# friendlymatthew/heif

Hardware: AMD Instinct MI355X
Metric: Mpixels/s decoded (bit-exact) on 4032x3024 HEIC batch (higher is better)
Workload: dtype u8

## Files before the change

### heif_amd/csrc/kernels/loopfilter.hip

```cpp
#include "kernels.hpp"

#include <algorithm>
#include <string>

namespace hg {

namespace {

__constant__ uint8_t c_beta[52] = {0,  0,  0,  0,  0,  0,  0,  0,  0,  0,  0,  0,  0,  0,  0,  0,  6,  7,
                                   8,  9,  10, 11, 12, 13, 14, 15, 16, 17, 18, 20, 22, 24, 26, 28, 30, 32,
                                   34, 36, 38, 40, 42, 44, 46, 48, 50, 52, 54, 56, 58, 60, 62, 64};
__constant__ uint8_t c_tc[54] = {0, 0, 0, 0, 0, 0, 0, 0, 0, 0, 0, 0, 0, 0, 0, 0, 0, 0, 1, 1, 1, 1, 1, 1, 1, 1, 1,
                                 2, 2, 2, 2, 3, 3, 3, 3, 4, 4, 4, 5, 5, 6, 6, 7, 8, 9, 10, 11, 13, 14, 16, 18, 20, 22, 24};

__device__ __forceinline__ int clip3(int lo, int hi, int v) { return v < lo ? lo : (v > hi ? hi : v); }

struct FastDiv {
    int d;
    float r;
    __device__ __forceinline__ explicit FastDiv(int d_) : d(d_ > 0 ? d_ : 1), r(1.0f / (float)(d_ > 0 ? d_ : 1)) {}
    __device__ __forceinline__ int div(int t, int &rem) const {
        int q = (int)((float)t * r);
        rem = t - q * d;
        if (rem < 0) {
            --q;
            rem += d;
        } else if (rem >= d) {
            ++q;
            rem -= d;
        }
        return q;
    }
};

__device__ __forceinline__ int chroma_qp_map(int qpi, int chroma) {
    if (chroma != 1) return qpi < 51 ? qpi : 51;
    if (qpi < 30) return qpi;
    if (qpi > 43) return qpi - 6;
    constexpr int t[14] = {29, 30, 31, 32, 33, 33, 34, 34, 35, 35, 36, 36, 37, 37};
    return t[qpi - 30];
}

template <typename Pel>
__device__ void luma_segment(Pel *q, int sx, int sk, int qpP, int qpQ, bool nofp, bool nofq, int beta_off,
                             int tc_off, int bd) {
#define PS(i, k) q[(k) * sk - ((i) + 1) * sx]
#define QS(i, k) q[(k) * sk + (i) * sx]
    const int qpl = (qpQ + qpP + 1) >> 1;
    const int beta = c_beta[clip3(0, 51, qpl + (beta_off << 1))] * (1 << (bd - 8));
    const int tc = c_tc[clip3(0, 53, qpl + 2 + (tc_off << 1))] * (1 << (bd - 8));
    const int dp0 = abs(PS(2, 0) - 2 * PS(1, 0) + PS(0, 0)), dp3 = abs(PS(2, 3) - 2 * PS(1, 3) + PS(0, 3));
    const int dq0 = abs(QS(2, 0) - 2 * QS(1, 0) + QS(0, 0)), dq3 = abs(QS(2, 3) - 2 * QS(1, 3) + QS(0, 3));
    const int dpq0 = dp0 + dq0, dpq3 = dp3 + dq3, dp = dp0 + dp3, dq = dq0 + dq3;
    if (dpq0 + dpq3 >= beta) return;
    auto dsam = [&](int k, int dpq) {
        return dpq < (beta >> 2) && abs(PS(3, k) - PS(0, k)) + abs(QS(0, k) - QS(3, k)) < (beta >> 3) &&
               abs(PS(0, k) - QS(0, k)) < ((5 * tc + 1) >> 1);
    };
    const bool strong = dsam(0, 2 * dpq0) && dsam(3, 2 * dpq3);
    const bool dEp = dp < ((beta + (beta >> 1)) >> 3), dEq = dq < ((beta + (beta >> 1)) >> 3);
    const int maxv = (1 << bd) - 1;
    for (int k = 0; k < 4; ++k) {
        const int p0 = PS(0, k), p1 = PS(1, k), p2 = PS(2, k), p3 = PS(3, k);
        const int q0 = QS(0, k), q1 = QS(1, k), q2 = QS(2, k), q3 = QS(3, k);
        if (strong) {
            if (!nofp) {
                PS(0, k) = (Pel)clip3(p0 - 2 * tc, p0 + 2 * tc, (p2 + 2 * p1 + 2 * p0 + 2 * q0 + q1 + 4) >> 3);
                PS(1, k) = (Pel)clip3(p1 - 2 * tc, p1 + 2 * tc, (p2 + p1 + p0 + q0 + 2) >> 2);
                PS(2, k) = (Pel)clip3(p2 - 2 * tc, p2 + 2 * tc, (2 * p3 + 3 * p2 + p1 + p0 + q0 + 4) >> 3);
            }
            if (!nofq) {
                QS(0, k) = (Pel)clip3(q0 - 2 * tc, q0 + 2 * tc, (p1 + 2 * p0 + 2 * q0 + 2 * q1 + q2 + 4) >> 3);
                QS(1, k) = (Pel)clip3(q1 - 2 * tc, q1 + 2 * tc, (p0 + q0 + q1 + q2 + 2) >> 2);
                QS(2, k) = (Pel)clip3(q2 - 2 * tc, q2 + 2 * tc, (p0 + q0 + q1 + 3 * q2 + 2 * q3 + 4) >> 3);
            }
        } else {
            int delta = (9 * (q0 - p0) - 3 * (q1 - p1) + 8) >> 4;
            if (abs(delta) < tc * 10) {
                delta = clip3(-tc, tc, delta);
                if (!nofp) PS(0, k) = (Pel)clip3(0, maxv, p0 + delta);
                if (!nofq) QS(0, k) = (Pel)clip3(0, maxv, q0 - delta);
                if (dEp && !nofp)
                    PS(1, k) = (Pel)clip3(0, maxv, p1 + clip3(-(tc >> 1), tc >> 1, (((p2 + p0 + 1) >> 1) - p1 + delta) >> 1));
                if (dEq && !nofq)
                    QS(1, k) = (Pel)clip3(0, maxv, q1 + clip3(-(tc >> 1), tc >> 1, (((q2 + q0 + 1) >> 1) - q1 - delta) >> 1));
            }
        }
    }
#undef PS
#undef QS
}

}

template <typename Pel>
__global__ void __launch_bounds__(256) k_assemble(BatchArgs a) {
    const int pic = a.pic0 + blockIdx.y;
    const PicDesc pd = a.pics[pic];
    if (!(pd.flags & PD_ASSEMBLY)) return;
    const SeqParams sp = a.seqs[pd.seq];
    const int W = sp.width, H = sp.height, w4 = (W + 3) >> 2, h4 = (H + 3) >> 2;
    const int wctb = (W + (1 << sp.log2_ctb) - 1) >> sp.log2_ctb;
    const int sx = chroma_sx(sp.chroma_format), sy = chroma_sy(sp.chroma_format);
    const int cw = sp.chroma_format ? W >> sx : 0, ch = sp.chroma_format ? H >> sy : 0;
    Pel *dY = reinterpret_cast<Pel *>(a.recon + pd.recon_off);
    uint8_t *dmap = a.maps + pd.map_off;
    const int tid = blockIdx.x * blockDim.x + threadIdx.x, nth = gridDim.x * blockDim.x;
    for (uint32_t c = 0; c < pd.nchild; ++c) {
        const PicDesc cd = a.pics[pd.child0 + c];
        const SeqParams cs = a.seqs[cd.seq];
        const int cW = cs.width, cH = cs.height, cw4 = (cW + 3) >> 2, ch4 = (cH + 3) >> 2;
        const int ccw = cs.chroma_format ? cW >> sx : 0, cch = cs.chroma_format ? cH >> sy : 0;
        const Pel *sY = reinterpret_cast<const Pel *>(a.recon + cd.recon_off);
        const int nl = cW * cH, nc = ccw * cch;
        for (int t = tid; t < nl + 2 * nc; t += nth) {
            if (t < nl) {
                const int x = t % cW, y = t / cW;
                dY[(size_t)(cd.org_y + y) * W + cd.org_x + x] = sY[t];
            } else {
                const int u = t - nl, k = u / nc, v = u % nc, x = v % ccw, y = v / ccw;
                dY[(size_t)W * H + (size_t)k * cw * ch + (size_t)((cd.org_y >> sy) + y) * cw + (cd.org_x >> sx) + x] = sY[t];
            }
        }
        const uint8_t *smap = a.maps + cd.map_off;
        const int nm = cw4 * ch4;
        for (int t = tid; t < 2 * nm; t += nth) {
            const int k = t / nm, v = t % nm, x = v % cw4, y = v / cw4;
            dmap[(size_t)k * w4 * h4 + (size_t)((cd.org_y >> 2) + y) * w4 + (cd.org_x >> 2) + x] = smap[t];
        }
        const int cwctb = (cW + (1 << cs.log2_ctb) - 1) >> cs.log2_ctb;
        const int chctb = (cH + (1 << cs.log2_ctb) - 1) >> cs.log2_ctb;
        const bool sao = cd.sao_luma || cd.sao_chroma;
        for (int t = tid; t < cwctb * chctb * 8; t += nth) {
            const int b = t >> 3, x = b % cwctb, y = b / cwctb;
            uint32_t *dst = reinterpret_cast<uint32_t *>(
                a.sao + pd.sao_off + (size_t)((cd.org_y >> sp.log2_ctb) + y) * wctb + (cd.org_x >> sp.log2_ctb) + x);
            dst[t & 7] = sao ? reinterpret_cast<const uint32_t *>(a.sao + cd.sao_off + b)[t & 7] : 0u;
        }
    }
    (void)h4;
}

template <typename Pel, bool VERT>
__global__ void __launch_bounds__(256) k_deblock(BatchArgs a) {
    const int pic = a.pic0 + blockIdx.y;
    const PicDesc pd = a.pics[pic];
    if (pd.dbk_disabled || (pd.flags & PD_CHILD)) return;
    const SeqParams sp = a.seqs[pd.seq];
    const int W = sp.width, H = sp.height;
    const int w4 = (W + 3) >> 2, h4 = (H + 3) >> 2;
    const int8_t *qpy = reinterpret_cast<const int8_t *>(a.maps + pd.map_off);
    const uint8_t *flg = a.maps + pd.map_off + (size_t)w4 * h4;
    Pel *Y = reinterpret_cast<Pel *>(a.recon + pd.recon_off);
    const int sx = chroma_sx(sp.chroma_format), sy = chroma_sy(sp.chroma_format);
    const int cw = sp.chroma_format ? W >> sx : 0, ch = sp.chroma_format ? H >> sy : 0;
    const int ne_l = VERT ? (W - 1) >> 3 : (H - 1) >> 3;
    const int ns_l = VERT ? H >> 2 : W >> 2;
    const int nl = ne_l * ns_l;
    const int ne_c = VERT ? (cw - 1) >> 3 : (ch - 1) >> 3;
    const int lc = VERT ? 4 >> sy : 4 >> sx;
    const int ns_c = VERT ? ch / lc : cw / lc;
    const int nc = sp.chroma_format ? ne_c * ns_c : 0;
    const int total = nl + 2 * nc;
    const FastDiv dl(VERT ? ne_l : ns_l), dc(nc), dce(VERT ? ne_c : ns_c);
    for (int t = blockIdx.x * blockDim.x + threadIdx.x; t < total; t += gridDim.x * blockDim.x) {
        if (t < nl) {
            int x, y, tr;
            const int tq = dl.div(t, tr);
            if (VERT) {
                x = 8 * (tr + 1);
                y = 4 * tq;
            } else {
                x = 4 * tr;
                y = 8 * (tq + 1);
            }
            const int fq = flg[(y >> 2) * w4 + (x >> 2)];
            if (!(fq & (VERT ? MF_EDGE_V : MF_EDGE_H))) continue;
            const int xp = VERT ? x - 1 : x, yp = VERT ? y : y - 1;
            const int fp = flg[(yp >> 2) * w4 + (xp >> 2)];
            luma_segment<Pel>(Y + (size_t)y * W + x, VERT ? 1 : W, VERT ? W : 1, qpy[(yp >> 2) * w4 + (xp >> 2)],
                              qpy[(y >> 2) * w4 + (x >> 2)], fp & MF_NOFILT, fq & MF_NOFILT, pd.beta_off, pd.tc_off,
                              sp.bit_depth_y);
        } else {
            const int u = t - nl;
            int v, vr;
            const int cidx = 1 + dc.div(u, v);
            const int vq = dce.div(v, vr);
            int xc, yc;
            if (VERT) {
                xc = 8 * (vr + 1);
                yc = lc * vq;
            } else {
                xc = lc * vr;
                yc = 8 * (vq + 1);
            }
            const int xl = xc << sx, yl = yc << sy;
            const int fq = flg[(yl >> 2) * w4 + (xl >> 2)];
            if (!(fq & (VERT ? MF_EDGE_V : MF_EDGE_H))) continue;
            const int xlp = VERT ? xl - 1 : xl, ylp = VERT ? yl : yl - 1;
            const int fp = flg[(ylp >> 2) * w4 + (xlp >> 2)];
            const int qpP = qpy[(ylp >> 2) * w4 + (xlp >> 2)], qpQ = qpy[(yl >> 2) * w4 + (xl >> 2)];
            const int off = cidx == 1 ? sp.cb_qp_offset : sp.cr_qp_offset;
            const int qpc = chroma_qp_map(((qpQ + qpP + 1) >> 1) + off, sp.chroma_format);
            const int bd = sp.bit_depth_c;
            const int tc = c_tc[clip3(0, 53, qpc + 2 + (pd.tc_off << 1))] * (1 << (bd - 8));
            const int maxv = (1 << bd) - 1;
            Pel *C = Y + (size_t)W * H + (size_t)(cidx - 1) * cw * ch;
            Pel *q = C + (size_t)yc * cw + xc;
            const int sa = VERT ? 1 : cw, sk = VERT ? cw : 1;
            for (int k = 0; k < lc; ++k) {
                const int p0 = q[k * sk - sa], p1 = q[k * sk - 2 * sa], q0 = q[k * sk], q1 = q[k * sk + sa];
                const int delta = clip3(-tc, tc, ((((q0 - p0) * 4) + p1 - q1 + 4) >> 3));
                if (!(fp & MF_NOFILT)) q[k * sk - sa] = (Pel)clip3(0, maxv, p0 + delta);
                if (!(fq & MF_NOFILT)) q[k * sk] = (Pel)clip3(0, maxv, q0 - delta);
            }
        }
    }
}

template <typename Pel>
__device__ __forceinline__ int sao_sample(const Pel *P, int PW, int PH, int xs, int ys, int cidx, int subx,
                                          int suby, const SaoParams *sao, int wctb, int log2ctb, const uint8_t *flg,
                                          int w4, int bd) {
    int v = P[(size_t)ys * PW + xs];
    const SaoParams &s = sao[(ys >> (log2ctb - suby)) * wctb + (xs >> (log2ctb - subx))];
    const int type = s.type[cidx];
    if (!type || (flg[((ys << suby) >> 2) * w4 + ((xs << subx) >> 2)] & MF_NOFILT)) return v;
    int o = 0;
    if (type == 2) {
        const int cl = s.band_eo[cidx];
        const int hx = cl == 0 ? 1 : (cl == 1 ? 0 : (cl == 2 ? 1 : -1));
        const int vy = cl == 0 ? 0 : 1;
        const int ax = xs - hx, ay = ys - vy, bx = xs + hx, by = ys + vy;
        if (ax >= 0 && ay >= 0 && ax < PW && ay < PH && bx >= 0 && by >= 0 && bx < PW && by < PH) {
            const int na = P[(size_t)ay * PW + ax], nb = P[(size_t)by * PW + bx];
            int e = 2 + (v > na) - (v < na) + (v > nb) - (v < nb);
            if (e <= 2) e = e == 2 ? 0 : e + 1;
            o = e ? s.off[cidx][e - 1] : 0;
        }
    } else {
        const int band = v >> (bd - 5);
        const int k = (band - s.band_eo[cidx]) & 31;
        o = k < 4 ? s.off[cidx][k] : 0;
    }
    return clip3(0, (1 << bd) - 1, v + o);
}

template <typename Pel>
struct QuadLoad;
template <>
struct QuadLoad<uint8_t> {
    using W = uint32_t;
    static __device__ __forceinline__ int at(W w, int j) { return (int)((w >> (8 * j)) & 0xffu); }
};
template <>
struct QuadLoad<uint16_t> {
    using W = uint64_t;
    static __device__ __forceinline__ int at(W w, int j) { return (int)((w >> (16 * j)) & 0xffffu); }
};

template <typename Pel>
__device__ __forceinline__ bool sao_quad(const Pel *P, int PW, int PH, int xs0, int ys, int cidx, int subx, int suby,
                                         const SaoParams *sao, int wctb, int log2ctb, const uint8_t *flg, int w4,
                                         int bd, int v[4]) {
    using Q = QuadLoad<Pel>;
    using W = typename Q::W;
    const Pel *row = P + (size_t)ys * PW;
    if ((xs0 & 3) || (PW & 3) || (reinterpret_cast<uintptr_t>(row + xs0) & (sizeof(W) - 1))) return false;
    const W c = *reinterpret_cast<const W *>(row + xs0);
#pragma unroll
    for (int j = 0; j < 4; ++j) v[j] = Q::at(c, j);
    const SaoParams &s = sao[(ys >> (log2ctb - suby)) * wctb + (xs0 >> (log2ctb - subx))];
    const int type = s.type[cidx];
    if (!type) return true;
    const uint8_t *fr = flg + (size_t)((ys << suby) >> 2) * w4;
    const int b0 = (xs0 << subx) >> 2, b3 = ((xs0 + 3) << subx) >> 2;
    const int f0 = fr[b0], f3 = fr[b3];
    const int cl = s.band_eo[cidx];
    const int maxv = (1 << bd) - 1;
    int o[4] = {0, 0, 0, 0};
    if (type == 2) {
        const int hx = cl == 0 ? 1 : (cl == 1 ? 0 : (cl == 2 ? 1 : -1)), vy = cl == 0 ? 0 : 1;
        const int ya = ys - vy, yb = ys + vy;
        const bool va = ya >= 0, vb = yb < PH;
        const Pel *ra = P + (size_t)(va ? ya : ys) * PW, *rb = P + (size_t)(vb ? yb : ys) * PW;
        const W qa = *reinterpret_cast<const W *>(ra + xs0), qb = *reinterpret_cast<const W *>(rb + xs0);
        const int xa_out = hx > 0 ? xs0 - 1 : xs0 + 4, xb_out = hx > 0 ? xs0 + 4 : xs0 - 1;
        const int ea = hx != 0 && xa_out >= 0 && xa_out < PW ? (int)ra[xa_out] : 0;
        const int eb = hx != 0 && xb_out >= 0 && xb_out < PW ? (int)rb[xb_out] : 0;
#pragma unroll
        for (int j = 0; j < 4; ++j) {
            const int ja = j - hx, jb = j + hx;
            const int na = ja < 0 || ja > 3 ? ea : Q::at(qa, ja < 0 ? 0 : (ja > 3 ? 3 : ja));
            const int nb = jb < 0 || jb > 3 ? eb : Q::at(qb, jb < 0 ? 0 : (jb > 3 ? 3 : jb));
            const bool in = va && vb && xs0 + ja >= 0 && xs0 + ja < PW && xs0 + jb >= 0 && xs0 + jb < PW;
            int e = 2 + (v[j] > na) - (v[j] < na) + (v[j] > nb) - (v[j] < nb);
            e = e <= 2 ? (e == 2 ? 0 : e + 1) : e;
            o[j] = in && e ? s.off[cidx][e - 1] : 0;
        }
    } else {
#pragma unroll
        for (int j = 0; j < 4; ++j) {
            const int k = ((v[j] >> (bd - 5)) - cl) & 31;
            o[j] = k < 4 ? s.off[cidx][k] : 0;
        }
    }
#pragma unroll
    for (int j = 0; j < 4; ++j) {
        const bool nf = ((((xs0 + j) << subx) >> 2) == b0 ? f0 : f3) & MF_NOFILT;
        if (!nf) v[j] = clip3(0, maxv, v[j] + o[j]);
    }
    return true;
}

template <typename Pel>
__global__ void __launch_bounds__(256) k_sao_out(BatchArgs a) {
    const int pic = a.pic0 + blockIdx.y;
    const PicDesc pd = a.pics[pic];
    if (pd.flags & PD_CHILD) return;
    const SeqParams sp = a.seqs[pd.seq];
    const OutImage oi = a.outs[pd.image];
    const int W = sp.width, H = sp.height, log2ctb = sp.log2_ctb;
    const int wctb = (W + (1 << log2ctb) - 1) >> log2ctb;
    const int w4 = (W + 3) >> 2, h4 = (H + 3) >> 2;
    const uint8_t *flg = a.maps + pd.map_off + (size_t)w4 * h4;
    const Pel *Y = reinterpret_cast<const Pel *>(a.recon + pd.recon_off);
    const int sx = chroma_sx(sp.chroma_format), sy = chroma_sy(sp.chroma_format);
    const int cw = sp.chroma_format ? W >> sx : 0, ch = sp.chroma_format ? H >> sy : 0;
    const SaoParams *sao = a.sao + pd.sao_off;
    const int vw = min(sp.out_w, oi.width - pd.out_x), vh = min(sp.out_h, oi.height - pd.out_y);
    if (vw <= 0 || vh <= 0) return;
    const int vcw = sp.chroma_format ? (vw + (1 << sx) - 1) >> sx : 0;
    const int vch = sp.chroma_format ? (vh + (1 << sy) - 1) >> sy : 0;
    const int qw = (vw + 3) >> 2, qcw = (vcw + 3) >> 2;
    const int nl = qw * vh, nc = qcw * vch;
    const int total = nl + 2 * nc;
    const FastDiv dq(qw), dn(nc), dqc(qcw);
    for (int t = blockIdx.x * blockDim.x + threadIdx.x; t < total; t += gridDim.x * blockDim.x) {
        int cidx, q, y;
        if (t < nl) {
            cidx = 0;
            y = dq.div(t, q);
        } else {
            const int u = t - nl;
            int v;
            cidx = 1 + dn.div(u, v);
            y = dqc.div(v, q);
        }
        const int subx = cidx ? sx : 0, suby = cidx ? sy : 0;
        const int PW = cidx ? cw : W, PH = cidx ? ch : H;
        const int vwc = cidx ? vcw : vw;
        const Pel *P = cidx == 0 ? Y : Y + (size_t)W * H + (size_t)(cidx - 1) * cw * ch;
        const int x0 = q * 4, n = min(4, vwc - x0);
        const int ys = y + (sp.conf_t >> suby), xs0 = x0 + (sp.conf_l >> subx);
        const bool on = pd.sao_luma || pd.sao_chroma;
        const int bd = cidx ? sp.bit_depth_c : sp.bit_depth_y;
        int v[4];
        if (!(n == 4 && on && sao_quad(P, PW, PH, xs0, ys, cidx, subx, suby, sao, wctb, log2ctb, flg, w4, bd, v))) {
#pragma unroll
            for (int j = 0; j < 4; ++j) {
                v[j] = 0;
                if (j < n)
                    v[j] = on ? sao_sample(P, PW, PH, xs0 + j, ys, cidx, subx, suby, sao, wctb, log2ctb, flg, w4, bd)
                              : (int)P[(size_t)ys * PW + xs0 + j];
            }
        }
        const uint64_t plane = cidx == 0 ? oi.plane[0] : (cidx == 1 ? oi.plane[1] : oi.plane[2]);
        const int pitch = cidx == 0 ? oi.pitch[0] : (cidx == 1 ? oi.pitch[1] : oi.pitch[2]);
        const int ox = (pd.out_x >> subx) + x0, oy = (pd.out_y >> suby) + y;
        Pel *dst = reinterpret_cast<Pel *>(plane + (size_t)oy * pitch) + ox;
        if (n == 4 && (reinterpret_cast<uintptr_t>(dst) & (4 * sizeof(Pel) - 1)) == 0) {
            if (sizeof(Pel) == 1)
                *reinterpret_cast<uint32_t *>(dst) = (uint32_t)v[0] | (uint32_t)v[1] << 8 | (uint32_t)v[2] << 16 |
                                                     (uint32_t)v[3] << 24;
            else
                *reinterpret_cast<uint64_t *>(dst) = (uint64_t)v[0] | (uint64_t)v[1] << 16 | (uint64_t)v[2] << 32 |
                                                     (uint64_t)v[3] << 48;
        } else {
            for (int j = 0; j < n; ++j) dst[j] = (Pel)v[j];
        }
    }
}


#if defined(HG_HOST_EMU)
void emu_deblock(const BatchArgs &a) {
    if (a.has_assembly) {
        if (a.bytes_per_sample == 1) emu_launch(k_assemble<uint8_t>, 1, a.n_pics, 1, a, true);
        else emu_launch(k_assemble<uint16_t>, 1, a.n_pics, 1, a, true);
    }
    if (a.bytes_per_sample == 1) {
        emu_launch(k_deblock<uint8_t, true>, 1, a.n_pics, 1, a, true);
        emu_launch(k_deblock<uint8_t, false>, 1, a.n_pics, 1, a, true);
    } else {
        emu_launch(k_deblock<uint16_t, true>, 1, a.n_pics, 1, a, true);
        emu_launch(k_deblock<uint16_t, false>, 1, a.n_pics, 1, a, true);
    }
}
void emu_sao_out(const BatchArgs &a) {
    if (a.bytes_per_sample == 1) emu_launch(k_sao_out<uint8_t>, 1, a.n_pics, 1, a, true);
    else emu_launch(k_sao_out<uint16_t>, 1, a.n_pics, 1, a, true);
}
#else
static int lf_blocks(int forced, int n_pics, int total, int lo, int hi) {
    int v = forced > 0 ? forced : total / (n_pics > 0 ? n_pics : 1);
    if (forced <= 0) v = v < lo ? lo : (v > hi ? hi : v);
    return v < 1 ? 1 : (v > 1024 ? 1024 : v);
}
static int env_int(const char *var) {
    const char *e = std::getenv(var);
    return e ? std::atoi(e) : 0;
}

hipError_t launch_deblock(const BatchArgs &a, hipStream_t s) {
    static const int forced = env_int("HEIFGPU_DBK_BLOCKS");
    dim3 grid(lf_blocks(forced, a.n_pics, 8192, 2, 64), a.n_pics), block(256);
    if (a.has_assembly) {
        if (a.bytes_per_sample == 1) hipLaunchKernelGGL(k_assemble<uint8_t>, grid, block, 0, s, a);
        else hipLaunchKernelGGL(k_assemble<uint16_t>, grid, block, 0, s, a);
    }
    if (a.bytes_per_sample == 1) {
        hipLaunchKernelGGL((k_deblock<uint8_t, true>), grid, block, 0, s, a);
        hipLaunchKernelGGL((k_deblock<uint8_t, false>), grid, block, 0, s, a);
    } else {
        hipLaunchKernelGGL((k_deblock<uint16_t, true>), grid, block, 0, s, a);
        hipLaunchKernelGGL((k_deblock<uint16_t, false>), grid, block, 0, s, a);
    }
    return hipGetLastError();
}

hipError_t launch_sao_out(const BatchArgs &a, hipStream_t s) {
    static const int forced = env_int("HEIFGPU_SAO_BLOCKS");
    dim3 grid(lf_blocks(forced, a.n_pics, 24576, 4, 256), a.n_pics), block(256);
    if (a.bytes_per_sample == 1) hipLaunchKernelGGL(k_sao_out<uint8_t>, grid, block, 0, s, a);
    else hipLaunchKernelGGL(k_sao_out<uint16_t>, grid, block, 0, s, a);
    return hipGetLastError();
}

__global__ void __launch_bounds__(256) k_status_fold(const uint32_t *__restrict__ st, uint32_t *__restrict__ sticky,
                                                     int n) {
    const int i = blockIdx.x * 256 + threadIdx.x;
    if (i < n) {
        const uint32_t v = st[i];
        if (v) sticky[i] |= v;
    }
}

hipError_t launch_status_fold(const uint32_t *status, uint32_t *sticky, int n, hipStream_t s) {
    if (n <= 0) return hipSuccess;
    hipLaunchKernelGGL(k_status_fold, dim3((n + 255) / 256), dim3(256), 0, s, status, sticky, n);
    return hipGetLastError();
}
#endif

}
```

Before: 28190.

## Vectorize SAO output kernel with 16-byte groups and packed 16-bit SIMD math

Rewrites the SAO-and-output kernel so each thread handles a 16-byte group of samples instead of 4 samples. It uses 128-bit loads and stores and packed 2x16-bit arithmetic through v_perm table lookups. The loop now runs per plane with a strided walk that avoids per-item division, and falls back to the old quad path for unaligned or tail columns. It also adds launch_bounds occupancy 8. The bit-exact edge and band offset logic now lives in new packed code, which adds correctness risk at picture edges and for the no-filter flags.

```diff
diff --git a/heif_amd/csrc/kernels/lf_pack.hpp b/heif_amd/csrc/kernels/lf_pack.hpp
--- /dev/null
+++ b/heif_amd/csrc/kernels/lf_pack.hpp
@@ -0,0 +1,115 @@
+#pragma once
+#include "wave.hpp"
+
+namespace hg {
+namespace lfp {
+
+#if !defined(HG_HOST_EMU)
+typedef short lf_s2 __attribute__((ext_vector_type(2)));
+typedef unsigned short lf_u2 __attribute__((ext_vector_type(2)));
+template <class V>
+__device__ __forceinline__ V lf_as(uint32_t a) {
+    V v;
+    __builtin_memcpy(&v, &a, 4);
+    return v;
+}
+template <class V>
+__device__ __forceinline__ uint32_t lf_word(V v) {
+    uint32_t a;
+    __builtin_memcpy(&a, &v, 4);
+    return a;
+}
+#endif
+
+__device__ __forceinline__ uint32_t pk_add(uint32_t a, uint32_t b) {
+#if defined(HG_HOST_EMU)
+    return ((a + b) & 0xffffu) | ((((a >> 16) + (b >> 16)) & 0xffffu) << 16);
+#else
+    return lf_word(lf_as<lf_u2>(a) + lf_as<lf_u2>(b));
+#endif
+}
+__device__ __forceinline__ uint32_t pk_sub(uint32_t a, uint32_t b) {
+#if defined(HG_HOST_EMU)
+    return ((a - b) & 0xffffu) | ((((a >> 16) - (b >> 16)) & 0xffffu) << 16);
+#else
+    return lf_word(lf_as<lf_u2>(a) - lf_as<lf_u2>(b));
+#endif
+}
+__device__ __forceinline__ uint32_t pk_max_i16(uint32_t a, uint32_t b) {
+#if defined(HG_HOST_EMU)
+    const int al = (int16_t)(a & 0xffffu), ah = (int16_t)(a >> 16), bl = (int16_t)(b & 0xffffu), bh = (int16_t)(b >> 16);
+    return (uint32_t)((al > bl ? al : bl) & 0xffff) | ((uint32_t)((ah > bh ? ah : bh) & 0xffff) << 16);
+#else
+    return lf_word(__builtin_elementwise_max(lf_as<lf_s2>(a), lf_as<lf_s2>(b)));
+#endif
+}
+__device__ __forceinline__ uint32_t pk_min_i16(uint32_t a, uint32_t b) {
+#if defined(HG_HOST_EMU)
+    const int al = (int16_t)(a & 0xffffu), ah = (int16_t)(a >> 16), bl = (int16_t)(b & 0xffffu), bh = (int16_t)(b >> 16);
+    return (uint32_t)((al < bl ? al : bl) & 0xffff) | ((uint32_t)((ah < bh ? ah : bh) & 0xffff) << 16);
+#else
+    return lf_word(__builtin_elementwise_min(lf_as<lf_s2>(a), lf_as<lf_s2>(b)));
+#endif
+}
+__device__ __forceinline__ uint32_t pk_ashr(uint32_t a, int n) {
+#if defined(HG_HOST_EMU)
+    const int al = (int16_t)(a & 0xffffu), ah = (int16_t)(a >> 16);
+    return (uint32_t)((al >> n) & 0xffff) | ((uint32_t)((ah >> n) & 0xffff) << 16);
+#else
+    return lf_word(lf_as<lf_s2>(a) >> (lf_s2){(short)n, (short)n});
+#endif
+}
+__device__ __forceinline__ uint32_t pk_lshr(uint32_t a, int n) {
+#if defined(HG_HOST_EMU)
+    return ((a & 0xffffu) >> n) | (((a >> 16) >> n) << 16);
+#else
+    return lf_word(lf_as<lf_u2>(a) >> (lf_u2){(unsigned short)n, (unsigned short)n});
+#endif
+}
+
+__device__ __forceinline__ uint32_t perm(uint32_t s0, uint32_t s1, uint32_t sel) {
+#if defined(HG_HOST_EMU)
+    const uint64_t in = ((uint64_t)s0 << 32) | s1;
+    uint32_t r = 0;
+    for (int k = 0; k < 4; ++k) {
+        const uint32_t s = (sel >> (8 * k)) & 0xffu;
+        uint32_t b;
+        if (s >= 13) b = 0xffu;
+        else if (s == 12) b = 0;
+        else if (s >= 8) b = ((in >> (16 * (s - 8) + 15)) & 1) ? 0xffu : 0u;
+        else b = (uint32_t)(in >> (8 * s)) & 0xffu;
+        r |= b << (8 * k);
+    }
+    return r;
+#else
+    return __builtin_amdgcn_perm(s0, s1, sel);
+#endif
+}
+
+__device__ __forceinline__ uint32_t pk_sign_diff(uint32_t a, uint32_t b) {
+    return pk_max_i16(pk_min_i16(pk_sub(a, b), 0x00010001u), 0xffffffffu);
+}
+
+__device__ __forceinline__ uint32_t pk_from_bytes(uint32_t w, int half) {
+    return perm(0, w, half ? 0x0c030c02u : 0x0c010c00u);
+}
+__device__ __forceinline__ uint32_t pk_to_bytes(uint32_t p0, uint32_t p1) { return perm(p1, p0, 0x06040200u); }
+
+__device__ __forceinline__ void sao_tables(uint32_t d1, uint32_t d2, uint32_t d3, bool edge, uint32_t &lo, uint32_t &hi) {
+    if (edge) {
+        lo = perm(d1, d2, 0x020c0006u);
+        hi = d3 & 0xffu;
+    } else {
+        lo = perm(d1, d2, 0x0c020006u) | (d3 << 24);
+        hi = 0;
+    }
+}
+__device__ __forceinline__ uint32_t sao_lookup(uint32_t lo, uint32_t hi, uint32_t idx) {
+    return pk_ashr(perm(hi, lo, (idx << 8) | 0x000c000cu), 8);
+}
+__device__ __forceinline__ uint32_t pk_add_clip(uint32_t c, uint32_t o, uint32_t maxv2) {
+    return pk_min_i16(pk_max_i16(pk_add(c, o), 0), maxv2);
+}
+
+}
+}
diff --git a/heif_amd/csrc/kernels/loopfilter.hip b/heif_amd/csrc/kernels/loopfilter.hip
--- a/heif_amd/csrc/kernels/loopfilter.hip
+++ b/heif_amd/csrc/kernels/loopfilter.hip
@@ -1,4 +1,5 @@
 #include "kernels.hpp"
+#include "lf_pack.hpp"
 
 #include <algorithm>
 #include <string>
@@ -314,7 +315,132 @@
 }
 
 template <typename Pel>
-__global__ void __launch_bounds__(256) k_sao_out(BatchArgs a) {
+__device__ __forceinline__ void sao_out_quad(const Pel *P, int PW, int PH, int xs0, int ys, int n, bool on, int cidx,
+                                             int subx, int suby, const SaoParams *sao, int wctb, int log2ctb,
+                                             const uint8_t *flg, int w4, int bd, Pel *dst) {
+    int v[4];
+    if (!(n == 4 && on && sao_quad(P, PW, PH, xs0, ys, cidx, subx, suby, sao, wctb, log2ctb, flg, w4, bd, v))) {
+#pragma unroll
+        for (int j = 0; j < 4; ++j) {
+            v[j] = 0;
+            if (j < n)
+                v[j] = on ? sao_sample(P, PW, PH, xs0 + j, ys, cidx, subx, suby, sao, wctb, log2ctb, flg, w4, bd)
+                          : (int)P[(size_t)ys * PW + xs0 + j];
+        }
+    }
+    if (n == 4 && (reinterpret_cast<uintptr_t>(dst) & (4 * sizeof(Pel) - 1)) == 0) {
+        if (sizeof(Pel) == 1)
+            *reinterpret_cast<uint32_t *>(dst) = (uint32_t)v[0] | (uint32_t)v[1] << 8 | (uint32_t)v[2] << 16 |
+                                                 (uint32_t)v[3] << 24;
+        else
+            *reinterpret_cast<uint64_t *>(dst) = (uint64_t)v[0] | (uint64_t)v[1] << 16 | (uint64_t)v[2] << 32 |
+                                                 (uint64_t)v[3] << 48;
+    } else {
+        for (int j = 0; j < n; ++j) dst[j] = (Pel)v[j];
+    }
+}
+
+struct alignas(16) Vec16 {
+    uint32_t w[4];
+};
+__device__ __forceinline__ Vec16 load16(const void *p) {
+    Vec16 v;
+    __builtin_memcpy(&v, __builtin_assume_aligned(p, 16), 16);
+    return v;
+}
+__device__ __forceinline__ void store16(void *p, const Vec16 &v) {
+    __builtin_memcpy(__builtin_assume_aligned(p, 16), &v, 16);
+}
+
+template <typename Pel>
+__device__ __forceinline__ uint32_t pack_of(const Vec16 &v, int p) {
+    if constexpr (sizeof(Pel) == 1) return lfp::pk_from_bytes(v.w[p >> 1], p & 1);
+    else return v.w[p];
+}
+
+template <typename Pel>
+__device__ __forceinline__ void sao_group(const Pel *P, int PW, int PH, int xs0, int ys, int cidx, int subx, int suby,
+                                          const SaoParams *sao, int wctb, int log2ctb, const uint8_t *flg, int w4,
+                                          int bd, Vec16 &out) {
+    using namespace lfp;
+    constexpr int G = 16 / (int)sizeof(Pel), BITS = 8 * (int)sizeof(Pel);
+    constexpr int NP = G / 2;
+    const Pel *row = P + (size_t)ys * PW + xs0;
+    const Vec16 c = load16(row);
+    out = c;
+    const uint32_t *sw =
+        reinterpret_cast<const uint32_t *>(sao + (ys >> (log2ctb - suby)) * wctb + (xs0 >> (log2ctb - subx)));
+    const uint64_t head = (uint64_t)sw[0] | (uint64_t)sw[1] << 32;
+    const int type = (int)(int8_t)(head >> (8 * cidx));
+    if (!type) return;
+    const int cl = (int)(head >> (24 + 8 * cidx)) & 0xff;
+    uint32_t tlo, thi;
+    sao_tables(sw[1 + 2 * cidx], sw[2 + 2 * cidx], sw[3 + 2 * cidx], type == 2, tlo, thi);
+    const uint32_t maxv2 = (uint32_t)((1 << bd) - 1) * 0x00010001u;
+    auto emit = [&](auto idx_of) {
+#pragma unroll
+        for (int i = 0; i < 4; ++i) {
+            if constexpr (sizeof(Pel) == 1) {
+                const uint32_t r0 = pk_add_clip(pack_of<Pel>(c, 2 * i), sao_lookup(tlo, thi, idx_of(2 * i)), maxv2);
+                const uint32_t r1 = pk_add_clip(pack_of<Pel>(c, 2 * i + 1), sao_lookup(tlo, thi, idx_of(2 * i + 1)), maxv2);
+                out.w[i] = pk_to_bytes(r0, r1);
+            } else {
+                out.w[i] = pk_add_clip(c.w[i], sao_lookup(tlo, thi, idx_of(i)), maxv2);
+            }
+        }
+    };
+    if (type == 2) {
+        const int vy = cl == 0 ? 0 : 1;
+        if (ys - vy < 0 || ys + vy >= PH) return;
+        const ptrdiff_t up = (ptrdiff_t)(cl >= 3 ? -vy : vy) * PW;
+        const Pel *rl = row - up, *rr = row + up;
+        Vec16 na = load16(rl), nb = load16(rr);
+        uint32_t first = 0xffffffffu, last = 0xffffffffu;
+        if (cl != 1) {
+            const uint32_t el = rl[xs0 > 0 ? -1 : 0], er = rr[xs0 + G < PW ? G : G - 1];
+            const Vec16 qa = na, qb = nb;
+            na.w[0] = (qa.w[0] << BITS) | el;
+            nb.w[3] = (qb.w[3] >> BITS) | (er << (32 - BITS));
+#pragma unroll
+            for (int i = 1; i < 4; ++i) {
+                na.w[i] = (qa.w[i] << BITS) | (qa.w[i - 1] >> (32 - BITS));
+                nb.w[i - 1] = (qb.w[i - 1] >> BITS) | (qb.w[i] << (32 - BITS));
+            }
+            if (xs0 == 0) first = 0xffff0000u;
+            if (xs0 + G == PW) last = 0x0000ffffu;
+        }
+        emit([&](int p) {
+            const uint32_t cp = pack_of<Pel>(c, p);
+            const uint32_t s = pk_add(pk_sign_diff(cp, pack_of<Pel>(na, p)), pk_sign_diff(cp, pack_of<Pel>(nb, p)));
+            return pk_add(p == 0 ? s & first : (p == NP - 1 ? s & last : s), 0x00020002u);
+        });
+    } else {
+        const uint32_t pos2 = (uint32_t)cl * 0x00010001u;
+        emit([&](int p) {
+            return pk_min_i16(pk_sub(pk_lshr(pack_of<Pel>(c, p), bd - 5), pos2) & 0x001f001fu, 0x00040004u);
+        });
+    }
+    const uint8_t *fr = flg + (size_t)((ys << suby) >> 2) * w4 + ((xs0 << subx) >> 2);
+    const int nf = (G << subx) >> 2;
+    uint64_t fw = 0;
+    if (nf == 8) __builtin_memcpy(&fw, fr, 8);
+    else if (nf == 4) __builtin_memcpy(&fw, fr, 4);
+    else __builtin_memcpy(&fw, fr, 2);
+    fw &= (uint64_t)MF_NOFILT * 0x0101010101010101ull;
+    if (fw) {
+#pragma unroll
+        for (int p = 0; p < NP; ++p) {
+            if ((fw >> (8 * (((2 * p) << subx) >> 2))) & 0xff) {
+                const int i = sizeof(Pel) == 1 ? p >> 1 : p;
+                const uint32_t m = sizeof(Pel) == 1 ? (p & 1 ? 0xffff0000u : 0x0000ffffu) : 0xffffffffu;
+                out.w[i] = (out.w[i] & ~m) | (c.w[i] & m);
+            }
+        }
+    }
+}
+
+template <typename Pel>
+__global__ void __launch_bounds__(256, 8) k_sao_out(BatchArgs a) {
     const int pic = a.pic0 + blockIdx.y;
     const PicDesc pd = a.pics[pic];
     if (pd.flags & PD_CHILD) return;
@@ -330,54 +456,56 @@
     const SaoParams *sao = a.sao + pd.sao_off;
     const int vw = min(sp.out_w, oi.width - pd.out_x), vh = min(sp.out_h, oi.height - pd.out_y);
     if (vw <= 0 || vh <= 0) return;
-    const int vcw = sp.chroma_format ? (vw + (1 << sx) - 1) >> sx : 0;
-    const int vch = sp.chroma_format ? (vh + (1 << sy) - 1) >> sy : 0;
-    const int qw = (vw + 3) >> 2, qcw = (vcw + 3) >> 2;
-    const int nl = qw * vh, nc = qcw * vch;
-    const int total = nl + 2 * nc;
-    const FastDiv dq(qw), dn(nc), dqc(qcw);
-    for (int t = blockIdx.x * blockDim.x + threadIdx.x; t < total; t += gridDim.x * blockDim.x) {
-        int cidx, q, y;
-        if (t < nl) {
-            cidx = 0;
-            y = dq.div(t, q);
-        } else {
-            const int u = t - nl;
-            int v;
-            cidx = 1 + dn.div(u, v);
-            y = dqc.div(v, q);
-        }
+    const bool on = pd.sao_luma || pd.sao_chroma;
+    constexpr int G = 16 / (int)sizeof(Pel), LOG2G = sizeof(Pel) == 1 ? 4 : 3;
+    const int tid = blockIdx.x * blockDim.x + threadIdx.x, nth = gridDim.x * blockDim.x;
+    for (int cidx = 0; cidx < (sp.chroma_format ? 3 : 1); ++cidx) {
         const int subx = cidx ? sx : 0, suby = cidx ? sy : 0;
         const int PW = cidx ? cw : W, PH = cidx ? ch : H;
-        const int vwc = cidx ? vcw : vw;
+        const int vwc = cidx ? (vw + (1 << sx) - 1) >> sx : vw, vhc = cidx ? (vh + (1 << sy) - 1) >> sy : vh;
         const Pel *P = cidx == 0 ? Y : Y + (size_t)W * H + (size_t)(cidx - 1) * cw * ch;
-        const int x0 = q * 4, n = min(4, vwc - x0);
-        const int ys = y + (sp.conf_t >> suby), xs0 = x0 + (sp.conf_l >> subx);
-        const bool on = pd.sao_luma || pd.sao_chroma;
         const int bd = cidx ? sp.bit_depth_c : sp.bit_depth_y;
-        int v[4];
-        if (!(n == 4 && on && sao_quad(P, PW, PH, xs0, ys, cidx, subx, suby, sao, wctb, log2ctb, flg, w4, bd, v))) {
-#pragma unroll
-            for (int j = 0; j < 4; ++j) {
-                v[j] = 0;
-                if (j < n)
-                    v[j] = on ? sao_sample(P, PW, PH, xs0 + j, ys, cidx, subx, suby, sao, wctb, log2ctb, flg, w4, bd)
-                              : (int)P[(size_t)ys * PW + xs0 + j];
-            }
-        }
+        const int cx0 = sp.conf_l >> subx, cy0 = sp.conf_t >> suby;
         const uint64_t plane = cidx == 0 ? oi.plane[0] : (cidx == 1 ? oi.plane[1] : oi.plane[2]);
         const int pitch = cidx == 0 ? oi.pitch[0] : (cidx == 1 ? oi.pitch[1] : oi.pitch[2]);
-        const int ox = (pd.out_x >> subx) + x0, oy = (pd.out_y >> suby) + y;
-        Pel *dst = reinterpret_cast<Pel *>(plane + (size_t)oy * pitch) + ox;
-        if (n == 4 && (reinterpret_cast<uintptr_t>(dst) & (4 * sizeof(Pel) - 1)) == 0) {
-            if (sizeof(Pel) == 1)
-                *reinterpret_cast<uint32_t *>(dst) = (uint32_t)v[0] | (uint32_t)v[1] << 8 | (uint32_t)v[2] << 16 |
-                                                     (uint32_t)v[3] << 24;
-            else
-                *reinterpret_cast<uint64_t *>(dst) = (uint64_t)v[0] | (uint64_t)v[1] << 16 | (uint64_t)v[2] << 32 |
-                                                     (uint64_t)v[3] << 48;
-        } else {
-            for (int j = 0; j < n; ++j) dst[j] = (Pel)v[j];
+        uint8_t *d0 = reinterpret_cast<uint8_t *>(plane) + (size_t)(pd.out_y >> suby) * pitch +
+                      (size_t)(pd.out_x >> subx) * sizeof(Pel);
+        const bool wide = (((PW * (int)sizeof(Pel)) | pitch) & 15) == 0 && (cx0 & (G - 1)) == 0 &&
+                          ((reinterpret_cast<uintptr_t>(P + cx0) | reinterpret_cast<uintptr_t>(d0)) & 15) == 0 &&
+                          log2ctb - subx >= LOG2G && bd <= 12;
+        const int gw = wide ? vwc >> LOG2G : 0;
+        if (gw > 0) {
+            const FastDiv dg(gw);
+            int g, y = dg.div(tid, g), dgr;
+            const int dy = dg.div(nth, dgr);
+            for (; y < vhc; y += dy) {
+                const int x0 = g << LOG2G, ys = y + cy0, xs0 = x0 + cx0;
+                Vec16 v;
+                if (on) sao_group<Pel>(P, PW, PH, xs0, ys, cidx, subx, suby, sao, wctb, log2ctb, flg, w4, bd, v);
+                else v = load16(P + (size_t)ys * PW + xs0);
+                store16(d0 + (size_t)y * pitch + (size_t)x0 * sizeof(Pel), v);
+                g += dgr;
+                if (g >= gw) {
+                    g -= gw;
+                    ++y;
+                }
+            }
+        }
+        const int xq = gw << LOG2G, qw = (vwc - xq + 3) >> 2;
+        if (qw > 0) {
+            const FastDiv dq(qw);
+            int q, y = dq.div(tid, q), dqr;
+            const int dy = dq.div(nth, dqr);
+            for (; y < vhc; y += dy) {
+                const int x0 = xq + 4 * q;
+                sao_out_quad<Pel>(P, PW, PH, x0 + cx0, y + cy0, min(4, vwc - x0), on, cidx, subx, suby, sao, wctb, log2ctb,
+                                  flg, w4, bd, reinterpret_cast<Pel *>(d0 + (size_t)y * pitch) + x0);
+                q += dqr;
+                if (q >= qw) {
+                    q -= qw;
+                    ++y;
+                }
+            }
         }
     }
 }
```

Measured after the change: 28670, median of 6. 1.7% higher.
